# ylsung/vl-merging

Measured on NVIDIA B200. Metric: gram_cache_samples_per_sec, higher is better.
Workload: dtype tf32

## Files before the change

vl-merging_b200/csrc/syrk_pair.cu:

```cuda
#include <algorithm>
#include <cstdlib>
#include <cstring>
#include <utility>
#include <map>
#include <mutex>
#include <tuple>
#include <type_traits>
#include <vector>

#include "common.cuh"
#include "syrk.h"
#include "umma.cuh"

namespace vlm {

namespace {

constexpr int kStagingBytes = 16384;
constexpr int kThreads = 256;
constexpr int kTmemCols = 512;
constexpr int kAccCols = 256;

__device__ __forceinline__ uint32_t cluster_ctarank() {
  uint32_t r;
  asm volatile("mov.u32 %0, %%cluster_ctarank;" : "=r"(r));
  return r;
}
__device__ __forceinline__ void cluster_sync_all() {
  asm volatile("barrier.cluster.arrive.release.aligned;" ::: "memory");
  asm volatile("barrier.cluster.wait.acquire.aligned;" ::: "memory");
}
__device__ __forceinline__ uint64_t l2_policy(int kind) {
  uint64_t p;
  if (kind == 1)
    asm volatile("createpolicy.fractional.L2::evict_first.b64 %0, 1.0;" : "=l"(p));
  else if (kind == 2)
    asm volatile("createpolicy.fractional.L2::evict_last.b64 %0, 1.0;" : "=l"(p));
  else
    asm volatile("createpolicy.fractional.L2::evict_normal.b64 %0, 1.0;" : "=l"(p));
  return p;
}
__device__ __forceinline__ void tma_reduce_add_2d_hint(const CUtensorMap* tm, const void* smem_src, int c0, int c1,
                                                       uint64_t pol) {
  asm volatile(
      "cp.reduce.async.bulk.tensor.2d.global.shared::cta.add.tile.bulk_group.L2::cache_hint [%0, {%2, %3}], [%1], %4;"
      ::"l"(reinterpret_cast<uint64_t>(tm)), "r"(smem_u32(smem_src)), "r"(c0), "r"(c1), "l"(pol)
      : "memory");
}

struct BatchSeg {
  int32_t sa, sb, k0, k1, pid, d, cps, pad;
};
__device__ __forceinline__ void tensormap_acquire(const CUtensorMap* tm) {
  asm volatile("fence.proxy.tensormap::generic.acquire.gpu [%0], 128;" ::"l"(reinterpret_cast<uint64_t>(tm)) : "memory");
}

}
}

#include "syrk_2sm.cuh"
#include "syrk_i8.cuh"

namespace vlm {
namespace {
struct DeviceSchedule2 {
  int nclusters = 0;
  PairSeg* d_segs = nullptr;
  int* d_off = nullptr;
};
std::mutex g_mu2;
typedef std::tuple<int, int64_t, int, int, int> ScheduleKey;
std::map<ScheduleKey, DeviceSchedule2> g_sched2;
std::vector<DeviceSchedule2> g_retired2;

template <typename Build>
int cached_schedule(const ScheduleKey& key, Build build, cudaStream_t stream, const DeviceSchedule2** out) {
  auto it = g_sched2.find(key);
  if (it == g_sched2.end()) {
    if (g_sched2.size() >= 512) {
      VLM_CUDA(cudaDeviceSynchronize());
      for (auto& ds : g_retired2) {
        cudaFree(ds.d_segs);
        cudaFree(ds.d_off);
      }
      g_retired2.clear();
      for (auto& kv : g_sched2) g_retired2.push_back(kv.second);
      g_sched2.clear();
    }
    std::vector<PairSeg> segs;
    std::vector<int> off;
    build(&segs, &off);
    DeviceSchedule2 ds;
    ds.nclusters = (int)off.size() - 1;
    VLM_CUDA(cudaMalloc(&ds.d_segs, std::max<size_t>(1, segs.size()) * sizeof(PairSeg)));
    VLM_CUDA(cudaMalloc(&ds.d_off, off.size() * sizeof(int)));
    VLM_CUDA(cudaMemcpyAsync(ds.d_segs, segs.data(), segs.size() * sizeof(PairSeg), cudaMemcpyHostToDevice, stream));
    VLM_CUDA(cudaMemcpyAsync(ds.d_off, off.data(), off.size() * sizeof(int), cudaMemcpyHostToDevice, stream));
    VLM_CUDA(cudaStreamSynchronize(stream));
    it = g_sched2.emplace(key, ds).first;
  }
  *out = &it->second;
  return 0;
}

inline int elem_bytes(int dtype) { return (dtype == VLM_F32 || dtype == VLM_TF32X2) ? 4 : 2; }
inline int chunk_rows(int dtype) { return dtype == VLM_TF32X2 ? 16 : 128 / elem_bytes(dtype); }

int encode_maps(EncodeTiledFn encode, const void* x, int dtype, int64_t rows, int d, int64_t ldx, int64_t seg_rows,
                int64_t seg_stride, float* g, int64_t ldg, CUtensorMap* tm_x, CUtensorMap* tm_g) {
  const int elem = elem_bytes(dtype);
  const int bk = chunk_rows(dtype), gc = 128 / elem;
  {
    const CUtensorMapDataType dt = elem == 4             ? CU_TENSOR_MAP_DATA_TYPE_TFLOAT32
                                   : dtype == VLM_BF16 ? CU_TENSOR_MAP_DATA_TYPE_BFLOAT16
                                                       : CU_TENSOR_MAP_DATA_TYPE_FLOAT16;
    const bool split = dtype == VLM_TF32X2;
    const bool segmented = !split && seg_rows > 0;
    const int rank = (split || segmented) ? 4 : 3;
    cuuint64_t gdim[4] = {(cuuint64_t)gc, (cuuint64_t)(segmented ? seg_rows : rows), (cuuint64_t)(d / gc),
                          (cuuint64_t)(split ? 2 : segmented ? rows / seg_rows : 1)};
    cuuint64_t gstr[3] = {(cuuint64_t)ldx * elem, 128, (cuuint64_t)(split ? rows * ldx : seg_stride) * elem};
    cuuint32_t box[4] = {(cuuint32_t)gc, (cuuint32_t)bk, (cuuint32_t)elem ,
                         (cuuint32_t)(split ? 2 : 1)};
    cuuint32_t estr[4] = {1, 1, 1, 1};
    const CUtensorMapSwizzle swz = elem == 4 ? CU_TENSOR_MAP_SWIZZLE_128B_ATOM_32B : CU_TENSOR_MAP_SWIZZLE_128B;
    CUresult r = encode(tm_x, dt, rank, const_cast<void*>(x), gdim, gstr, box, estr, CU_TENSOR_MAP_INTERLEAVE_NONE, swz,
                        CU_TENSOR_MAP_L2_PROMOTION_L2_256B, CU_TENSOR_MAP_FLOAT_OOB_FILL_NONE);
    VLM_REQUIRE(r == CUDA_SUCCESS, VLM_ERR_DRIVER, "cuTensorMapEncodeTiled(X, %d-D) failed: CUresult %d", rank, (int)r);
  }
  {
    cuuint64_t gdim[2] = {(cuuint64_t)d, (cuuint64_t)d};
    cuuint64_t gstr[1] = {(cuuint64_t)ldg * 4};
    cuuint32_t box[2] = {32, 128};
    cuuint32_t estr[2] = {1, 1};
    CUresult r = encode(tm_g, CU_TENSOR_MAP_DATA_TYPE_FLOAT32, 2, g, gdim, gstr, box, estr, CU_TENSOR_MAP_INTERLEAVE_NONE,
                        CU_TENSOR_MAP_SWIZZLE_128B, CU_TENSOR_MAP_L2_PROMOTION_NONE, CU_TENSOR_MAP_FLOAT_OOB_FILL_NONE);
    VLM_REQUIRE(r == CUDA_SUCCESS, VLM_ERR_DRIVER, "cuTensorMapEncodeTiled(G) failed: CUresult %d", (int)r);
  }
  return 0;
}

struct Scratch {
  void* ptr[4] = {nullptr, nullptr, nullptr, nullptr};
  size_t cap[4] = {0, 0, 0, 0};
  int next = 0;
};
std::map<std::pair<int, cudaStream_t>, Scratch> g_scratch;

int l2_hints() {
  static const int v = [] {
    const char* e = getenv("VLM_SYRK_L2_HINTS");
    return e ? atoi(e) : (2 << 2);
  }();
  return v;
}

typedef void (*PairKernel)(const CUtensorMap, const CUtensorMap, const CUtensorMap*, const void*, const int*, int, int,
                           int);
template <bool BATCH>
PairKernel pick_kernel(int dtype) {
  if (dtype == VLM_TF32X2) return syrk_2sm_kernel<4, 2, BATCH, true>;
  if (dtype == VLM_F32) return syrk_2sm_kernel<4, 2, BATCH, false>;
  if (dtype == VLM_BF16) return syrk_2sm_kernel<2, 1, BATCH, false>;
  return syrk_2sm_kernel<2, 0, BATCH, false>;
}

}

void build_pair_schedule(int64_t kc, int d, int nclusters_max, std::vector<PairSeg>* segs, std::vector<int>* off,
                         int64_t seg_cap_arg, int64_t min_piece_arg) {
  int64_t seg_cap = seg_cap_arg > 0 ? seg_cap_arg : 128;
  if (const char* e = getenv("VLM_SYRK_SEG_CHUNKS")) seg_cap = std::max(1, atoi(e));
  const int nsb = (d + 255) / 256;
  struct T {
    int a, b;
  };
  std::vector<T> tiles;
  for (int a = 0; a < nsb; ++a)
    for (int b = a; b < nsb; ++b) tiles.push_back({a, b});
  const int64_t ntile = (int64_t)tiles.size();
  const int64_t min_chunks = 8;
  const int C = nclusters_max;
  std::vector<std::vector<PairSeg>> per;
  auto emit = [&](int c, const T& t, int64_t k0, int64_t k1) {
    if (k1 <= k0) return;
    const int64_t pieces = (k1 - k0 + seg_cap - 1) / seg_cap;
    for (int64_t i = 0; i < pieces; ++i) {
      const int64_t a = k0 + (k1 - k0) * i / pieces, b = k0 + (k1 - k0) * (i + 1) / pieces;
      per[c].push_back({t.a, t.b, (int)a, (int)b});
    }
  };
  per.resize(C);
  const int64_t rounds = ntile / C;
  for (int64_t r = 0; r < rounds; ++r)
    for (int c = 0; c < C; ++c) emit(c, tiles[r * C + c], 0, kc);
  const int64_t rem = ntile - rounds * C;
  if (rem > 0) {
    const int64_t p_lo = std::max<int64_t>(1, (kc + seg_cap - 1) / seg_cap);
    const int64_t min_piece = min_piece_arg > 0 ? min_piece_arg : (kc >= 8 * 64 ? 64 : min_chunks);
    const int64_t p_hi = std::max<int64_t>(p_lo, kc / min_piece);
    int64_t best_p = p_lo;
    double best = 1e30;
    for (int64_t p = p_lo; p <= p_hi; ++p) {
      const double makespan = (double)((rem * p + C - 1) / C) / (double)p;
      if (makespan < best - 1e-9) best = makespan, best_p = p;
    }
    std::vector<std::vector<PairSeg>> sweep;
    static const bool interleave_on = [] {
      const char* e = getenv("VLM_SYRK_INTERLEAVE");
      return e ? atoi(e) != 0 : true;
    }();
    const bool interleave = interleave_on && rounds > 0;
    if (interleave) {
      sweep.resize(C);
      for (int c = 0; c < C; ++c) {
        const size_t n_last = (size_t)((kc + seg_cap - 1) / seg_cap);
        sweep[c].assign(per[c].end() - n_last, per[c].end());
        per[c].resize(per[c].size() - n_last);
      }
    }
    int64_t q = 0;
    for (int64_t p = 0; p < best_p; ++p)
      for (int64_t t = 0; t < rem; ++t, ++q)
        emit((int)(q % C), tiles[rounds * C + t], kc * p / best_p, kc * (p + 1) / best_p);
    if (interleave) {
      for (int c = 0; c < C; ++c) {
        const size_t n_before = (size_t)(rounds - 1) * (size_t)((kc + seg_cap - 1) / seg_cap);
        std::vector<PairSeg> pieces(per[c].begin() + n_before, per[c].end());
        per[c].resize(n_before);
        size_t i = 0;
        for (const PairSeg& own : sweep[c]) {
          per[c].push_back(own);
          while (i < pieces.size() && pieces[i].k0 < own.k1) per[c].push_back(pieces[i++]);
        }
        while (i < pieces.size()) per[c].push_back(pieces[i++]);
      }
    }
  }
  while (!per.empty() && per.back().empty()) per.pop_back();
  segs->clear();
  off->assign(1, 0);
  for (auto& v : per) {
    segs->insert(segs->end(), v.begin(), v.end());
    off->push_back((int)segs->size());
  }
}

void build_syrk_pair_schedule_host(int64_t kc, int d, int nsm, std::vector<int32_t>* flat, std::vector<int>* off) {
  std::vector<PairSeg> segs;
  build_pair_schedule(kc, d, nsm / 2, &segs, off);
  flat->clear();
  for (const PairSeg& s : segs) {
    flat->push_back(s.sa);
    flat->push_back(s.sb);
    flat->push_back(s.k0);
    flat->push_back(s.k1);
  }
}

static void build_i8_schedule(int64_t kc, int d, int C, std::vector<PairSeg>* segs, std::vector<int>* off);
void build_syrk_i8_schedule_host(int64_t kc, int d, int nsm, std::vector<int32_t>* flat, std::vector<int>* off) {
  std::vector<PairSeg> segs;
  build_i8_schedule(kc, d, nsm / 2, &segs, off);
  flat->clear();
  for (const PairSeg& s : segs) {
    flat->push_back(s.sa);
    flat->push_back(s.sb);
    flat->push_back(s.k0);
    flat->push_back(s.k1);
  }
}

bool syrk_pair_supported(int dtype, const void* x, int d, int64_t ldx, int64_t seg_stride, const float* g, int64_t ldg) {
  const int elem = elem_bytes(dtype);
  return d % (128 / elem) == 0 &&
         (reinterpret_cast<uintptr_t>(x) & 15) == 0 && ((ldx * elem) & 15) == 0 && ((seg_stride * elem) & 15) == 0 &&
         (reinterpret_cast<uintptr_t>(g) & 15) == 0 && (ldg & 3) == 0;
}

static inline void seg_chunks(int64_t rows, int64_t seg_rows, int bk, int64_t* cps, int64_t* kc) {
  if (seg_rows > 0) {
    *cps = (seg_rows + bk - 1) / bk;
    *kc = (rows / seg_rows) * *cps;
  } else {
    *cps = 0;
    *kc = (rows + bk - 1) / bk;
  }
}

int syrk_pair_launch(const void* x, int dtype, int64_t rows, int d, int64_t ldx, int64_t seg_rows, int64_t seg_stride,
                    float* g, int64_t ldg, cudaStream_t stream) {
  const int bk = chunk_rows(dtype);
  VLM_REQUIRE(rows < (int64_t)1 << 31, VLM_ERR_INVALID_ARG, "vlm_syrk_accum: rows too large");
  if (seg_rows >= rows || dtype == VLM_TF32X2) seg_rows = 0;
  int dev = 0, nsm = 0;
  VLM_CUDA(cudaGetDevice(&dev));
  if (int rc = device_sm_count(&nsm)) return rc;
  EncodeTiledFn encode = nullptr;
  if (int rc = tensor_map_encoder(&encode)) return rc;
  int64_t cps, kc;
  seg_chunks(rows, seg_rows, bk, &cps, &kc);
  VLM_REQUIRE(kc < (int64_t)1 << 30, VLM_ERR_INVALID_ARG, "vlm_syrk_accum: too many row chunks");
  CUtensorMap tm_x, tm_g;
  if (int rc = encode_maps(encode, x, dtype, rows, d, ldx, seg_rows, seg_stride, g, ldg, &tm_x, &tm_g)) return rc;
  const int smem = k2SmemBytes;
  PairKernel kernel = pick_kernel<false>(dtype);

  std::lock_guard<std::mutex> lk(g_mu2);
  const DeviceSchedule2* sched = nullptr;
  if (int rc = cached_schedule(std::make_tuple(dev, kc, d, bk, nsm),
                               [&](std::vector<PairSeg>* segs, std::vector<int>* off) {
                                 build_pair_schedule(kc, d, nsm / 2, segs, off);
                               },
                               stream, &sched))
    return rc;
  VLM_CUDA(cudaFuncSetAttribute(kernel, cudaFuncAttributeMaxDynamicSharedMemorySize, smem));
  kernel<<<2 * sched->nclusters, kThreads, smem, stream>>>(tm_x, tm_g, nullptr, sched->d_segs, sched->d_off, d, (int)cps,
                                                           l2_hints());
  VLM_CUDA(cudaGetLastError());
  count_launch();
  return 0;
}

int tf32_split_launch(const float* x, int64_t rows, int d, int64_t ldx, int64_t seg_rows, int64_t seg_stride, float* out,
                      cudaStream_t stream) {
  int nsm = 0;
  if (int rc = device_sm_count(&nsm)) return rc;
  if (seg_rows >= rows) seg_rows = 0;
  const int64_t n4 = rows * (d / 4);
  const int64_t blocks = std::min<int64_t>((n4 + 255) / 256, (int64_t)nsm * 8);
  tf32_split_kernel<<<(unsigned)std::max<int64_t>(1, blocks), 256, 0, stream>>>(x, rows, d, ldx, seg_rows, seg_stride, out);
  VLM_CUDA(cudaGetLastError());
  count_launch();
  return 0;
}

size_t syrk_i8x4_scratch_bytes(int64_t rows, int d) { return (size_t)4 * rows * d + (size_t)8 * d + 64; }

static void build_i8_schedule(int64_t kc, int d, int C, std::vector<PairSeg>* segs, std::vector<int>* off) {
  const int nsb = (d + 255) / 256;
  const int T = nsb * (nsb + 1) / 2;
  segs->clear();
  off->assign(1, 0);
  const int m = (int)std::min<int64_t>(C / T, kc / 6);
  if (m >= 3 && kc >= 64) {
    const double w[3] = {7.0, 5.0, 1.15};
    const double fixed = 200.0;
    int best[3] = {0, 0, 0};
    double best_t = 1e30;
    for (int n0 = 1; n0 <= m - 2; ++n0)
      for (int n1 = 1; n0 + n1 <= m - 1; ++n1) {
        const int n2 = m - n0 - n1;
        const double t = std::max(w[0] / n0, std::max(w[1] / n1, w[2] / n2));
        if (t < best_t - 1e-12) best_t = t, best[0] = n0, best[1] = n1, best[2] = n2;
      }
    const double t_split = best_t * (double)kc + fixed;
    const double t_all = (w[0] + w[1] + w[2]) / m * (double)kc + 3 * fixed;
    if (t_split < t_all) {
      for (int a = 0; a < nsb; ++a)
        for (int b = a; b < nsb; ++b)
          for (int ph = 0; ph < kI8Phases; ++ph)
            for (int i = 0; i < best[ph]; ++i) {
              const int64_t g = ph == 2 ? 4 : 1, units = (kc + g - 1) / g;
              const int64_t k0 = std::min(kc, units * i / best[ph] * g), k1 = std::min(kc, units * (i + 1) / best[ph] * g);
              if (k1 > k0) {
                for (int64_t k = k0; k < k1; k += 2048)
                  segs->push_back({a, b | (ph << 16), (int)k, (int)std::min(k1, k + 2048)});
                off->push_back((int)segs->size());
              }
            }
      return;
    }
  }
  std::vector<PairSeg> base;
  std::vector<int> boff;
  build_pair_schedule(kc, d, C, &base, &boff, 2048);
  for (size_t c = 0; c + 1 < boff.size(); ++c) {
    for (int i = boff[c]; i < boff[c + 1]; ++i)
      for (int ph = 0; ph < kI8Phases; ++ph) segs->push_back({base[i].sa, base[i].sb | (ph << 16), base[i].k0, base[i].k1});
    off->push_back((int)segs->size());
  }
}

template <typename T>
static int i8_prepass(const T* x, int64_t rows, int d, int64_t ldx, int64_t seg_rows, int64_t seg_stride, unsigned* amax,
                      int* exps, int8_t* planes, int nsm, cudaStream_t stream) {
  VLM_CUDA(cudaMemsetAsync(amax, 0, sizeof(unsigned) * d, stream));
  const int64_t slabs = std::max<int64_t>(1, std::min<int64_t>((rows + 255) / 256, (int64_t)nsm * 16 / std::max(1, d / 128)));
  const int64_t rps = (rows + slabs - 1) / slabs;
  i8_colmax_kernel<T><<<dim3((unsigned)(d / 128), (unsigned)((rows + rps - 1) / rps)), 256, 0, stream>>>(
      x, rows, d, ldx, seg_rows, seg_stride, rps, amax);
  i8_exps_kernel<<<(d + 255) / 256, 256, 0, stream>>>(amax, d, exps);
  i8_slice_kernel<T><<<(unsigned)std::max<int64_t>(1, std::min<int64_t>(rows, (int64_t)nsm * 4)), 256, 0, stream>>>(
      x, rows, d, ldx, seg_rows, seg_stride, reinterpret_cast<const float*>(amax), planes);
  VLM_CUDA(cudaGetLastError());
  count_launch(3);
  return 0;
}

int syrk_i8x4_launch(const void* x, int dtype, int64_t rows, int d, int64_t ldx, int64_t seg_rows, int64_t seg_stride,
                     void* scratch, double* g, int64_t ldg, cudaStream_t stream) {
  int dev = 0, nsm = 0;
  VLM_CUDA(cudaGetDevice(&dev));
  if (int rc = device_sm_count(&nsm)) return rc;
  EncodeTiledFn encode = nullptr;
  if (int rc = tensor_map_encoder(&encode)) return rc;
  if (seg_rows >= rows) seg_rows = 0;
  int8_t* planes = static_cast<int8_t*>(scratch);
  int* exps = reinterpret_cast<int*>(planes + (((size_t)4 * rows * d + 15) & ~(size_t)15));
  unsigned* amax = reinterpret_cast<unsigned*>(exps + d);
  int rc;
  if (dtype == VLM_F32)
    rc = i8_prepass(static_cast<const float*>(x), rows, d, ldx, seg_rows, seg_stride, amax, exps, planes, nsm, stream);
  else if (dtype == VLM_F16)
    rc = i8_prepass(static_cast<const __half*>(x), rows, d, ldx, seg_rows, seg_stride, amax, exps, planes, nsm, stream);
  else
    rc = i8_prepass(static_cast<const __nv_bfloat16*>(x), rows, d, ldx, seg_rows, seg_stride, amax, exps, planes, nsm, stream);
  if (rc) return rc;

  CUtensorMap tm_p[3];
  for (int ph = 0; ph < 3; ++ph) {
    const cuuint32_t np = ph == 0 ? 4 : ph == 1 ? 3 : 1;
    cuuint64_t gdim[4] = {128, (cuuint64_t)rows, (cuuint64_t)(d / 128), np};
    cuuint64_t gstr[3] = {(cuuint64_t)d, 128, (cuuint64_t)rows * d};
    cuuint32_t box[4] = {128, (cuuint32_t)(ph == 2 ? 128 : 32), 1, np};
    cuuint32_t estr[4] = {1, 1, 1, 1};
    CUresult r = encode(&tm_p[ph], CU_TENSOR_MAP_DATA_TYPE_UINT8, 4, planes, gdim, gstr, box, estr,
                        CU_TENSOR_MAP_INTERLEAVE_NONE, CU_TENSOR_MAP_SWIZZLE_128B, CU_TENSOR_MAP_L2_PROMOTION_L2_256B,
                        CU_TENSOR_MAP_FLOAT_OOB_FILL_NONE);
    VLM_REQUIRE(r == CUDA_SUCCESS, VLM_ERR_DRIVER, "cuTensorMapEncodeTiled(int8 planes) failed: CUresult %d", (int)r);
  }
  CUtensorMap tm_g;
  {
    cuuint64_t gdim[2] = {(cuuint64_t)d, (cuuint64_t)d};
    cuuint64_t gstr[1] = {(cuuint64_t)ldg * 8};
    cuuint32_t box[2] = {16, 128};
    cuuint32_t estr[2] = {1, 1};
    CUresult r = encode(&tm_g, CU_TENSOR_MAP_DATA_TYPE_FLOAT64, 2, g, gdim, gstr, box, estr, CU_TENSOR_MAP_INTERLEAVE_NONE,
                        CU_TENSOR_MAP_SWIZZLE_128B, CU_TENSOR_MAP_L2_PROMOTION_NONE, CU_TENSOR_MAP_FLOAT_OOB_FILL_NONE);
    VLM_REQUIRE(r == CUDA_SUCCESS, VLM_ERR_DRIVER, "cuTensorMapEncodeTiled(G fp64) failed: CUresult %d", (int)r);
  }
  const int64_t kc = (rows + 31) / 32;
  VLM_REQUIRE(kc < (int64_t)1 << 30, VLM_ERR_INVALID_ARG, "vlm_syrk_accum_i8x4: too many row chunks");
  std::lock_guard<std::mutex> lk(g_mu2);
  const DeviceSchedule2* sched = nullptr;
  if (int rc = cached_schedule(std::make_tuple(dev, kc, d, -8, nsm),
                               [&](std::vector<PairSeg>* segs, std::vector<int>* off) {
                                 build_i8_schedule(kc, d, nsm / 2, segs, off);
                               },
                               stream, &sched))
    return rc;
  const int smem = kI8SmemBytes;
  VLM_CUDA(cudaFuncSetAttribute(syrk_i8x4_kernel, cudaFuncAttributeMaxDynamicSharedMemorySize, smem));
  I8Args args{g, ldg, exps};
  syrk_i8x4_kernel<<<2 * sched->nclusters, kThreads, smem, stream>>>(tm_p[0], tm_p[1], tm_p[2], tm_g, sched->d_segs,
                                                                     sched->d_off, d, args);
  VLM_CUDA(cudaGetLastError());
  count_launch();
  return 0;
}

int syrk_pair_batch_launch(const vlm_syrk_problem* probs, int n, int dtype, cudaStream_t stream) {
  const int bk = chunk_rows(dtype);
  int dev = 0, nsm = 0;
  VLM_CUDA(cudaGetDevice(&dev));
  if (int rc = device_sm_count(&nsm)) return rc;
  EncodeTiledFn encode = nullptr;
  if (int rc = tensor_map_encoder(&encode)) return rc;
  const int C = nsm / 2;
  std::vector<CUtensorMap> maps(2 * (size_t)n);
  std::vector<std::vector<BatchSeg>> per(C);
  std::vector<int64_t> load(C, 0);
  struct ShapeSched {
    std::vector<PairSeg> segs;
    std::vector<int> off;
    std::vector<std::pair<int64_t, int>> shares;
  };
  std::map<std::pair<int64_t, int>, ShapeSched> by_shape;
  int64_t batch_work = 0;
  for (int p = 0; p < n; ++p) {
    const int64_t nsb = (probs[p].d + 255) / 256;
    batch_work += nsb * (nsb + 1) / 2 * ((probs[p].rows + bk - 1) / bk);
  }
  const int64_t min_piece = batch_work >= (int64_t)8 * 64 * C ? 64 : 0;
  for (int p = 0; p < n; ++p) {
    const vlm_syrk_problem& q = probs[p];
    VLM_REQUIRE(q.rows < (int64_t)1 << 31, VLM_ERR_INVALID_ARG, "vlm_syrk_accum: rows too large");
    const int64_t seg_rows = (dtype != VLM_TF32X2 && q.seg_rows > 0 && q.seg_rows < q.rows) ? q.seg_rows : 0;
    if (int rc = encode_maps(encode, q.x, dtype, q.rows, q.d, q.ldx, seg_rows, q.seg_stride, q.g, q.ldg, &maps[2 * p],
                             &maps[2 * p + 1]))
      return rc;
    int64_t cps, kc;
    seg_chunks(q.rows, seg_rows, bk, &cps, &kc);
    auto found = by_shape.find({kc, q.d});
    if (found == by_shape.end()) {
      ShapeSched ss;
      build_pair_schedule(kc, q.d, C, &ss.segs, &ss.off, 0, min_piece);
      for (int c = 0; c + 1 < (int)ss.off.size(); ++c) {
        int64_t cost = 0;
        for (int s = ss.off[c]; s < ss.off[c + 1]; ++s) cost += ss.segs[s].k1 - ss.segs[s].k0;
        ss.shares.push_back({cost, c});
      }
      std::sort(ss.shares.begin(), ss.shares.end(),
                [](auto& a, auto& b) { return a.first > b.first || (a.first == b.first && a.second < b.second); });
      found = by_shape.emplace(std::make_pair(kc, q.d), std::move(ss)).first;
    }
    const std::vector<PairSeg>& segs = found->second.segs;
    const std::vector<int>& off = found->second.off;
    const std::vector<std::pair<int64_t, int>>& shares = found->second.shares;
    std::vector<int> order(C);
    for (int c = 0; c < C; ++c) order[c] = c;
    std::stable_sort(order.begin(), order.end(), [&](int a, int b) { return load[a] < load[b]; });
    for (size_t i = 0; i < shares.size(); ++i) {
      const int dst = order[i % C], c = shares[i].second;
      for (int s = off[c]; s < off[c + 1]; ++s)
        per[dst].push_back({segs[s].sa, segs[s].sb, segs[s].k0, segs[s].k1, p, q.d, (int)cps, 0});
      load[dst] += shares[i].first;
    }
  }
  int ncl = C;
  while (ncl > 0 && per[ncl - 1].empty()) --ncl;
  std::vector<BatchSeg> flat;
  std::vector<int> foff(1, 0);
  for (int c = 0; c < ncl; ++c) {
    flat.insert(flat.end(), per[c].begin(), per[c].end());
    foff.push_back((int)flat.size());
  }
  if (flat.empty()) return 0;
  const size_t maps_bytes = maps.size() * sizeof(CUtensorMap);
  const size_t off_bytes = ((foff.size() * sizeof(int)) + 127) / 128 * 128;
  const size_t seg_bytes = flat.size() * sizeof(BatchSeg);
  const size_t total = maps_bytes + off_bytes + seg_bytes;
  std::vector<uint8_t> host(total);
  memcpy(host.data(), maps.data(), maps_bytes);
  memcpy(host.data() + maps_bytes, foff.data(), foff.size() * sizeof(int));
  memcpy(host.data() + maps_bytes + off_bytes, flat.data(), seg_bytes);
  uint8_t* dptr = nullptr;
  {
    std::lock_guard<std::mutex> lk(g_mu2);
    Scratch& sc = g_scratch[{dev, stream}];
    const int i = sc.next;
    sc.next = (sc.next + 1) % 4;
    if (sc.cap[i] < total) {
      if (sc.ptr[i]) VLM_CUDA(cudaFree(sc.ptr[i]));
      sc.cap[i] = std::max<size_t>(total * 2, 1 << 18);
      VLM_CUDA(cudaMalloc(&sc.ptr[i], sc.cap[i]));
    }
    dptr = static_cast<uint8_t*>(sc.ptr[i]);
  }
  VLM_CUDA(cudaMemcpyAsync(dptr, host.data(), total, cudaMemcpyHostToDevice, stream));
  const int smem = k2SmemBytes;
  PairKernel kernel = pick_kernel<true>(dtype);
  VLM_CUDA(cudaFuncSetAttribute(kernel, cudaFuncAttributeMaxDynamicSharedMemorySize, smem));
  kernel<<<2 * ncl, kThreads, smem, stream>>>(maps[0], maps[1], reinterpret_cast<const CUtensorMap*>(dptr),
                                              dptr + maps_bytes + off_bytes,
                                              reinterpret_cast<const int*>(dptr + maps_bytes), 0, 0, l2_hints());
  VLM_CUDA(cudaGetLastError());
  count_launch();
  return 0;
}

}
```

Before: 1218.

## Cache batch schedules globally, pin staging buffers, and skip redundant smem attribute calls

The batched path now reuses per-shape pair schedules across calls through the global schedule cache instead of rebuilding them each call. It also stages uploads in pinned host slots guarded by events, so the memcpy is truly asynchronous and no temporary vector is allocated. cudaFuncSetAttribute is called once per kernel and device rather than on every launch. The aim is lower host-side launch overhead, at the cost of holding g_mu2 across the whole scheduling loop and extra pinned memory.

```diff
diff --git a/vl-merging_b200/csrc/syrk_pair.cu b/vl-merging_b200/csrc/syrk_pair.cu
--- a/vl-merging_b200/csrc/syrk_pair.cu
+++ b/vl-merging_b200/csrc/syrk_pair.cu
@@ -4,6 +4,7 @@
 #include <utility>
 #include <map>
 #include <mutex>
+#include <set>
 #include <tuple>
 #include <type_traits>
 #include <vector>
@@ -63,18 +64,21 @@
 
 namespace vlm {
 namespace {
-struct DeviceSchedule2 {
+struct CachedSchedule {
   int nclusters = 0;
   PairSeg* d_segs = nullptr;
   int* d_off = nullptr;
+  std::vector<PairSeg> segs;
+  std::vector<int> off;
+  std::vector<std::pair<int64_t, int>> shares;
 };
 std::mutex g_mu2;
-typedef std::tuple<int, int64_t, int, int, int> ScheduleKey;
-std::map<ScheduleKey, DeviceSchedule2> g_sched2;
-std::vector<DeviceSchedule2> g_retired2;
+typedef std::tuple<int, int64_t, int, int, int, int64_t> ScheduleKey;
+std::map<ScheduleKey, CachedSchedule> g_sched2;
+std::vector<CachedSchedule> g_retired2;
 
 template <typename Build>
-int cached_schedule(const ScheduleKey& key, Build build, cudaStream_t stream, const DeviceSchedule2** out) {
+int cached_schedule(const ScheduleKey& key, Build build, bool upload, cudaStream_t stream, const CachedSchedule** out) {
   auto it = g_sched2.find(key);
   if (it == g_sched2.end()) {
     if (g_sched2.size() >= 512) {
@@ -84,22 +88,45 @@
         cudaFree(ds.d_off);
       }
       g_retired2.clear();
-      for (auto& kv : g_sched2) g_retired2.push_back(kv.second);
+      for (auto& kv : g_sched2) g_retired2.push_back(std::move(kv.second));
       g_sched2.clear();
     }
-    std::vector<PairSeg> segs;
-    std::vector<int> off;
-    build(&segs, &off);
-    DeviceSchedule2 ds;
-    ds.nclusters = (int)off.size() - 1;
-    VLM_CUDA(cudaMalloc(&ds.d_segs, std::max<size_t>(1, segs.size()) * sizeof(PairSeg)));
-    VLM_CUDA(cudaMalloc(&ds.d_off, off.size() * sizeof(int)));
-    VLM_CUDA(cudaMemcpyAsync(ds.d_segs, segs.data(), segs.size() * sizeof(PairSeg), cudaMemcpyHostToDevice, stream));
-    VLM_CUDA(cudaMemcpyAsync(ds.d_off, off.data(), off.size() * sizeof(int), cudaMemcpyHostToDevice, stream));
-    VLM_CUDA(cudaStreamSynchronize(stream));
-    it = g_sched2.emplace(key, ds).first;
+    CachedSchedule ds;
+    build(&ds.segs, &ds.off);
+    ds.nclusters = (int)ds.off.size() - 1;
+    if (upload) {
+      VLM_CUDA(cudaMalloc(&ds.d_segs, std::max<size_t>(1, ds.segs.size()) * sizeof(PairSeg)));
+      VLM_CUDA(cudaMalloc(&ds.d_off, ds.off.size() * sizeof(int)));
+      VLM_CUDA(cudaMemcpyAsync(ds.d_segs, ds.segs.data(), ds.segs.size() * sizeof(PairSeg), cudaMemcpyHostToDevice,
+                               stream));
+      VLM_CUDA(cudaMemcpyAsync(ds.d_off, ds.off.data(), ds.off.size() * sizeof(int), cudaMemcpyHostToDevice, stream));
+      VLM_CUDA(cudaStreamSynchronize(stream));
+      ds.segs.clear();
+      ds.segs.shrink_to_fit();
+      ds.off.clear();
+      ds.off.shrink_to_fit();
+    } else {
+      for (int c = 0; c < ds.nclusters; ++c) {
+        int64_t cost = 0;
+        for (int s = ds.off[c]; s < ds.off[c + 1]; ++s) cost += ds.segs[s].k1 - ds.segs[s].k0;
+        ds.shares.push_back({cost, c});
+      }
+      std::sort(ds.shares.begin(), ds.shares.end(),
+                [](auto& a, auto& b) { return a.first > b.first || (a.first == b.first && a.second < b.second); });
+    }
+    it = g_sched2.emplace(key, std::move(ds)).first;
   }
   *out = &it->second;
+  return 0;
+}
+
+int raise_smem_limit(const void* kernel, int smem, int dev) {
+  static std::mutex mu;
+  static std::set<std::pair<const void*, int>> done;
+  std::lock_guard<std::mutex> lk(mu);
+  if (done.count({kernel, dev})) return 0;
+  VLM_CUDA(cudaFuncSetAttribute(kernel, cudaFuncAttributeMaxDynamicSharedMemorySize, smem));
+  done.insert({kernel, dev});
   return 0;
 }
 
@@ -140,12 +167,15 @@
   return 0;
 }
 
-struct Scratch {
-  void* ptr[4] = {nullptr, nullptr, nullptr, nullptr};
-  size_t cap[4] = {0, 0, 0, 0};
+struct Staging {
+  static constexpr int kSlots = 8;
+  uint8_t* host[kSlots] = {};
+  void* dev[kSlots] = {};
+  size_t cap[kSlots] = {};
+  cudaEvent_t uploaded[kSlots] = {};
   int next = 0;
 };
-std::map<std::pair<int, cudaStream_t>, Scratch> g_scratch;
+std::map<std::pair<int, cudaStream_t>, Staging> g_staging;
 
 int l2_hints() {
   static const int v = [] {
@@ -307,14 +337,14 @@
   PairKernel kernel = pick_kernel<false>(dtype);
 
   std::lock_guard<std::mutex> lk(g_mu2);
-  const DeviceSchedule2* sched = nullptr;
-  if (int rc = cached_schedule(std::make_tuple(dev, kc, d, bk, nsm),
+  const CachedSchedule* sched = nullptr;
+  if (int rc = cached_schedule(std::make_tuple(dev, kc, d, bk, nsm, (int64_t)-1),
                                [&](std::vector<PairSeg>* segs, std::vector<int>* off) {
                                  build_pair_schedule(kc, d, nsm / 2, segs, off);
                                },
-                               stream, &sched))
+                               true, stream, &sched))
     return rc;
-  VLM_CUDA(cudaFuncSetAttribute(kernel, cudaFuncAttributeMaxDynamicSharedMemorySize, smem));
+  if (int rc = raise_smem_limit(reinterpret_cast<const void*>(kernel), smem, dev)) return rc;
   kernel<<<2 * sched->nclusters, kThreads, smem, stream>>>(tm_x, tm_g, nullptr, sched->d_segs, sched->d_off, d, (int)cps,
                                                            l2_hints());
   VLM_CUDA(cudaGetLastError());
@@ -443,15 +473,15 @@
   const int64_t kc = (rows + 31) / 32;
   VLM_REQUIRE(kc < (int64_t)1 << 30, VLM_ERR_INVALID_ARG, "vlm_syrk_accum_i8x4: too many row chunks");
   std::lock_guard<std::mutex> lk(g_mu2);
-  const DeviceSchedule2* sched = nullptr;
-  if (int rc = cached_schedule(std::make_tuple(dev, kc, d, -8, nsm),
+  const CachedSchedule* sched = nullptr;
+  if (int rc = cached_schedule(std::make_tuple(dev, kc, d, -8, nsm, (int64_t)-1),
                                [&](std::vector<PairSeg>* segs, std::vector<int>* off) {
                                  build_i8_schedule(kc, d, nsm / 2, segs, off);
                                },
-                               stream, &sched))
+                               true, stream, &sched))
     return rc;
   const int smem = kI8SmemBytes;
-  VLM_CUDA(cudaFuncSetAttribute(syrk_i8x4_kernel, cudaFuncAttributeMaxDynamicSharedMemorySize, smem));
+  if (int rc = raise_smem_limit(reinterpret_cast<const void*>(syrk_i8x4_kernel), smem, dev)) return rc;
   I8Args args{g, ldg, exps};
   syrk_i8x4_kernel<<<2 * sched->nclusters, kThreads, smem, stream>>>(tm_p[0], tm_p[1], tm_p[2], tm_g, sched->d_segs,
                                                                      sched->d_off, d, args);
@@ -471,18 +501,13 @@
   std::vector<CUtensorMap> maps(2 * (size_t)n);
   std::vector<std::vector<BatchSeg>> per(C);
   std::vector<int64_t> load(C, 0);
-  struct ShapeSched {
-    std::vector<PairSeg> segs;
-    std::vector<int> off;
-    std::vector<std::pair<int64_t, int>> shares;
-  };
-  std::map<std::pair<int64_t, int>, ShapeSched> by_shape;
   int64_t batch_work = 0;
   for (int p = 0; p < n; ++p) {
     const int64_t nsb = (probs[p].d + 255) / 256;
     batch_work += nsb * (nsb + 1) / 2 * ((probs[p].rows + bk - 1) / bk);
   }
   const int64_t min_piece = batch_work >= (int64_t)8 * 64 * C ? 64 : 0;
+  std::lock_guard<std::mutex> lk(g_mu2);
   for (int p = 0; p < n; ++p) {
     const vlm_syrk_problem& q = probs[p];
     VLM_REQUIRE(q.rows < (int64_t)1 << 31, VLM_ERR_INVALID_ARG, "vlm_syrk_accum: rows too large");
@@ -492,22 +517,16 @@
       return rc;
     int64_t cps, kc;
     seg_chunks(q.rows, seg_rows, bk, &cps, &kc);
-    auto found = by_shape.find({kc, q.d});
-    if (found == by_shape.end()) {
-      ShapeSched ss;
-      build_pair_schedule(kc, q.d, C, &ss.segs, &ss.off, 0, min_piece);
-      for (int c = 0; c + 1 < (int)ss.off.size(); ++c) {
-        int64_t cost = 0;
-        for (int s = ss.off[c]; s < ss.off[c + 1]; ++s) cost += ss.segs[s].k1 - ss.segs[s].k0;
-        ss.shares.push_back({cost, c});
-      }
-      std::sort(ss.shares.begin(), ss.shares.end(),
-                [](auto& a, auto& b) { return a.first > b.first || (a.first == b.first && a.second < b.second); });
-      found = by_shape.emplace(std::make_pair(kc, q.d), std::move(ss)).first;
-    }
-    const std::vector<PairSeg>& segs = found->second.segs;
-    const std::vector<int>& off = found->second.off;
-    const std::vector<std::pair<int64_t, int>>& shares = found->second.shares;
+    const CachedSchedule* sched = nullptr;
+    if (int rc = cached_schedule(std::make_tuple(dev, kc, q.d, bk, nsm, min_piece),
+                                 [&](std::vector<PairSeg>* segs, std::vector<int>* off) {
+                                   build_pair_schedule(kc, q.d, C, segs, off, 0, min_piece);
+                                 },
+                                 false, stream, &sched))
+      return rc;
+    const std::vector<PairSeg>& segs = sched->segs;
+    const std::vector<int>& off = sched->off;
+    const std::vector<std::pair<int64_t, int>>& shares = sched->shares;
     std::vector<int> order(C);
     for (int c = 0; c < C; ++c) order[c] = c;
     std::stable_sort(order.begin(), order.end(), [&](int a, int b) { return load[a] < load[b]; });
@@ -520,38 +539,43 @@
   }
   int ncl = C;
   while (ncl > 0 && per[ncl - 1].empty()) --ncl;
-  std::vector<BatchSeg> flat;
-  std::vector<int> foff(1, 0);
+  size_t nseg = 0;
+  for (int c = 0; c < ncl; ++c) nseg += per[c].size();
+  if (nseg == 0) return 0;
+  const size_t maps_bytes = maps.size() * sizeof(CUtensorMap);
+  const size_t off_bytes = (((size_t)(ncl + 1) * sizeof(int)) + 127) / 128 * 128;
+  const size_t total = maps_bytes + off_bytes + nseg * sizeof(BatchSeg);
+  Staging& st = g_staging[{dev, stream}];
+  const int i = st.next;
+  st.next = (st.next + 1) % Staging::kSlots;
+  if (st.uploaded[i]) VLM_CUDA(cudaEventSynchronize(st.uploaded[i]));
+  else VLM_CUDA(cudaEventCreateWithFlags(&st.uploaded[i], cudaEventDisableTiming));
+  if (st.cap[i] < total) {
+    if (st.dev[i]) VLM_CUDA(cudaFree(st.dev[i]));
+    if (st.host[i]) VLM_CUDA(cudaFreeHost(st.host[i]));
+    st.dev[i] = nullptr;
+    st.host[i] = nullptr;
+    st.cap[i] = 0;
+    const size_t cap = std::max<size_t>(total * 2, 1 << 18);
+    VLM_CUDA(cudaMalloc(&st.dev[i], cap));
+    VLM_CUDA(cudaMallocHost(&st.host[i], cap));
+    st.cap[i] = cap;
+  }
+  uint8_t* host = st.host[i];
+  uint8_t* dptr = static_cast<uint8_t*>(st.dev[i]);
+  memcpy(host, maps.data(), maps_bytes);
+  int* foff = reinterpret_cast<int*>(host + maps_bytes);
+  BatchSeg* flat = reinterpret_cast<BatchSeg*>(host + maps_bytes + off_bytes);
+  foff[0] = 0;
   for (int c = 0; c < ncl; ++c) {
-    flat.insert(flat.end(), per[c].begin(), per[c].end());
-    foff.push_back((int)flat.size());
-  }
-  if (flat.empty()) return 0;
-  const size_t maps_bytes = maps.size() * sizeof(CUtensorMap);
-  const size_t off_bytes = ((foff.size() * sizeof(int)) + 127) / 128 * 128;
-  const size_t seg_bytes = flat.size() * sizeof(BatchSeg);
-  const size_t total = maps_bytes + off_bytes + seg_bytes;
-  std::vector<uint8_t> host(total);
-  memcpy(host.data(), maps.data(), maps_bytes);
-  memcpy(host.data() + maps_bytes, foff.data(), foff.size() * sizeof(int));
-  memcpy(host.data() + maps_bytes + off_bytes, flat.data(), seg_bytes);
-  uint8_t* dptr = nullptr;
-  {
-    std::lock_guard<std::mutex> lk(g_mu2);
-    Scratch& sc = g_scratch[{dev, stream}];
-    const int i = sc.next;
-    sc.next = (sc.next + 1) % 4;
-    if (sc.cap[i] < total) {
-      if (sc.ptr[i]) VLM_CUDA(cudaFree(sc.ptr[i]));
-      sc.cap[i] = std::max<size_t>(total * 2, 1 << 18);
-      VLM_CUDA(cudaMalloc(&sc.ptr[i], sc.cap[i]));
-    }
-    dptr = static_cast<uint8_t*>(sc.ptr[i]);
-  }
-  VLM_CUDA(cudaMemcpyAsync(dptr, host.data(), total, cudaMemcpyHostToDevice, stream));
+    std::copy(per[c].begin(), per[c].end(), flat + foff[c]);
+    foff[c + 1] = foff[c] + (int)per[c].size();
+  }
+  VLM_CUDA(cudaMemcpyAsync(dptr, host, total, cudaMemcpyHostToDevice, stream));
+  VLM_CUDA(cudaEventRecord(st.uploaded[i], stream));
   const int smem = k2SmemBytes;
   PairKernel kernel = pick_kernel<true>(dtype);
-  VLM_CUDA(cudaFuncSetAttribute(kernel, cudaFuncAttributeMaxDynamicSharedMemorySize, smem));
+  if (int rc = raise_smem_limit(reinterpret_cast<const void*>(kernel), smem, dev)) return rc;
   kernel<<<2 * ncl, kThreads, smem, stream>>>(maps[0], maps[1], reinterpret_cast<const CUtensorMap*>(dptr),
                                               dptr + maps_bytes + off_bytes,
                                               reinterpret_cast<const int*>(dptr + maps_bytes), 0, 0, l2_hints());
```

Result: no change. 1215 (median of 6 runs) (-0.3%).
